# tmoroney/whisper-diarize-rs

Measured on AMD Instinct MI355X. Metric: audio-sec/wall-sec (xRT), large-v3 + DTW + diarize, 1/2/4/8 MI355X, higher is better.
Workload: dtype f16 (f32 accumulate)

## Files before the change

include/wdr.h:

```cpp
#ifndef WDR_H
#define WDR_H

#include <stddef.h>
#include <stdint.h>

#ifdef __cplusplus
extern "C" {
#endif

#define WDR_ABI_VERSION 6

typedef struct wdr_engine wdr_engine;
typedef struct wdr_context wdr_context;

typedef struct {
  const char* cache_dir;
  int8_t enable_dtw;
  int8_t enable_flash_attn;
  int8_t use_gpu;
  int8_t has_gpu_device;
  int32_t gpu_device;
  const char* vad_model_path;
  const char* diarize_segment_model_path;
  const char* diarize_embedding_model_path;
// ... 202 lines not shown
                          uint64_t chunk_frames, int32_t host, int16_t** out, size_t* n_out, double* ms);
int wdr_dbg_audio_split(const uint8_t* raw, uint64_t n_frames, int32_t fmt, int32_t channels, int32_t rate,
                        uint64_t chunk_frames, int32_t host, int16_t** out, size_t* n_per_channel, double* ms);
int wdr_dbg_resample_table(int32_t rate, int32_t* L, int32_t* M, int32_t* T, float** tab);
int wdr_dbg_mfma_scale(const uint8_t* a, const uint8_t* b, const int32_t* sa, const int32_t* sb, float* out);
int wdr_dbg_encode(wdr_context* c, const float* mel_window , float* enc_out );
int wdr_dbg_cross_kv(wdr_context* c, float* out);
int wdr_dbg_decode(wdr_context* c, const int32_t* tokens, size_t n, float* logits_out );
int wdr_dbg_step(wdr_context* c, const int32_t* tokens, size_t n, float* logits_out );
int wdr_dbg_logits(wdr_context* c, const float* logits, int32_t R, const int32_t* ctl, const float* temperature,
                   float max_initial_ts, int32_t suppress_blank, int32_t* ids_out, float* f_out);
int wdr_dbg_batch_step(wdr_context* c, const int32_t* tokens, size_t n, int32_t rows, int32_t iters,
                       double* ms_per_step);
int wdr_dbg_capture(wdr_context* c, const int32_t* tokens, size_t n, float* cap_out );
int wdr_dbg_dtw(const float* cap, int32_t n_heads, int32_t n_tok, int32_t n_audio, int32_t sot_len, int32_t seek,
                float* x_out , int32_t* times_out, int32_t* n_times);
int wdr_dbg_discrete(const float* w, size_t n, uint32_t seed, int32_t n_draws, int32_t* out);
int wdr_dbg_dtw_dp(const float* x, int32_t rows, int32_t cols, int32_t seek, int32_t* times_out, int32_t* n_times);
int wdr_dbg_proj_fp8(const uint16_t* a_f16, const uint16_t* w_f16, const float* bias, int32_t M, int32_t N, int32_t K,
                     int32_t epi, float* out, uint8_t* a8_out, uint8_t* a_scale_out, uint8_t* w8_out,
                     uint8_t* w_scale_out);
int wdr_dbg_proj(const uint16_t* a_f16, const uint16_t* w_f16, const float* bias, int32_t M, int32_t N, int32_t K,
                 int32_t epi, float* out );
#define WDR_DBG_PROJ_ROWS 0x200
#define WDR_DBG_PROJ_GEMM1 0x800
#define WDR_DBG_PROJ_PACKED 0x1000
int wdr_dbg_pack_rows(const uint16_t* w_f16, int32_t N, int32_t K, uint16_t* out);
int wdr_dbg_proj_ln(const float* x, const float* gamma, const float* beta, const uint16_t* w_f16, const float* bias,
                    int32_t M, int32_t N, int32_t K, int32_t epi, int32_t fused, float* out);
int wdr_dbg_attn(const uint16_t* q, const uint16_t* k, const uint16_t* v, int32_t Tq, int32_t Tk, int32_t n_head,
                 int32_t causal, float* out );
int wdr_dbg_xattn(const uint16_t* q, const uint16_t* kv, const int32_t* row_slot, const int32_t* grp, int32_t R,
                  int32_t S, int32_t H, int32_t iters, float* out);

int wdr_dbg_self_attn(const uint16_t* q, const uint16_t* kc, const uint16_t* vc, int32_t n_seq, int32_t T,
                      const int32_t* row_seq, const int32_t* row_pos, int32_t R, int32_t H, float* out);
int wdr_dbg_proj_qkv(const uint16_t* a_f16, const uint16_t* w_f16, const float* bias, int32_t M, int32_t d, int32_t K,
                     const int32_t* row_seq, const int32_t* row_pos, int32_t n_seq, int32_t T, uint16_t* kc_io,
                     uint16_t* vc_io, float* q_out);
int wdr_dbg_proj_qkv_packed(const uint16_t* a_f16, const uint16_t* w_f16, const float* bias, int32_t M, int32_t d,
                            int32_t K, const int32_t* row_seq, const int32_t* row_pos, int32_t n_seq, int32_t T,
                            uint16_t* kc_io, uint16_t* vc_io, float* q_out);
int wdr_dbg_logits_topk(wdr_context* c, const float* logits, int32_t R, const int32_t* ctl, const float* temperature,
                        float max_initial_ts, int32_t suppress_blank, int32_t K, int32_t* ids_out, float* f_out);
int wdr_dbg_logits_probs(wdr_context* c, const float* logits, int32_t R, const int32_t* ctl, const float* temperature,
                         float max_initial_ts, int32_t suppress_blank, float* probs_out, float* logprobs_out);
int wdr_dbg_kv_rows(wdr_context* c, int32_t seq, int32_t n_rows, int32_t write, uint16_t* k, uint16_t* v);
int wdr_dbg_kv_reorder(wdr_context* c, const int32_t* src, const int32_t* dst, int32_t n, int32_t n_rows);

#ifdef __cplusplus
}
#endif
#endif
```

whisper-diarize-rs_amd/csrc/engine.cpp:

```cpp
#include <algorithm>
#include <atomic>
#include <chrono>
#include <cmath>
#include <cstdio>
#include <cstdlib>
#include <cstring>
#include <fstream>
#include <map>
#include <memory>
#include <random>
#include <string>
#include <sys/stat.h>
#include <dirent.h>
#include <condition_variable>
#include <exception>
#include <mutex>
#include <set>
#include <pthread.h>
#include <thread>
#include <vector>

#include "../../include/wdr.h"
#include "audio_file.h"
#include "audio_gpu.h"
// ... 2480 lines not shown
      WDR_HIP(hipMemcpy(h.data(), dout.p, h.size() * 2, hipMemcpyDeviceToHost));
      for (size_t i = 0; i < h.size(); ++i) out[i] = (float)h[i];
    }
    return 0;
  })
}

int wdr_dbg_attn(const uint16_t* q, const uint16_t* k, const uint16_t* v, int32_t Tq, int32_t Tk, int32_t H,
                 int32_t causal, float* out) {
  WDR_GUARD({
    const int d = H * 64;
    DevMem dq((size_t)Tq * d * 2), dk((size_t)Tk * d * 2), dv((size_t)Tk * d * 2), dout((size_t)Tq * d * 2);
    WDR_HIP(hipMemcpy(dq.p, q, dq.bytes, hipMemcpyHostToDevice));
    WDR_HIP(hipMemcpy(dk.p, k, dk.bytes, hipMemcpyHostToDevice));
    WDR_HIP(hipMemcpy(dv.p, v, dv.bytes, hipMemcpyHostToDevice));
    FlashArgs fa{dq.as<f16>(), d, 0, dk.as<f16>(), d, 0, dv.as<f16>(), d, 0, dout.as<f16>(), d, 0, nullptr, Tq, Tk, H,
                 causal, 0.125f};
    DevMem po, pml;
    if (!causal && Tq <= 256 && Tk >= 512) {
      fa.nsplit = 12;
      po = DevMem((size_t)12 * Tq * H * 64 * 4);
      pml = DevMem((size_t)12 * H * Tq * 8);
      fa.part_o = po.as<float>();
      fa.part_ml = pml.as<float2>();
    }
    launch_flash_attn(fa, 1, nullptr);
    std::vector<f16> h((size_t)Tq * d);
    WDR_HIP(hipMemcpy(h.data(), dout.p, h.size() * 2, hipMemcpyDeviceToHost));
    for (size_t i = 0; i < h.size(); ++i) out[i] = (float)h[i];
    return 0;
  })
}

int wdr_dbg_xattn(const uint16_t* q, const uint16_t* kv, const int32_t* row_slot, const int32_t* grp, int32_t R,
                  int32_t S, int32_t H, int32_t iters, float* out) {
  WDR_GUARD({
    WDR_CHECK(R >= 1 && R <= 1024 && S >= 1 && H >= 1 && H <= 32 && iters >= 1, "dbg xattn: bad shape");
    const int d = H * 64, T = 1500;
    DevMem dq((size_t)R * d * 2), dkv((size_t)S * T * 2 * d * 2), dout((size_t)R * d * 2);
    DevMem po((size_t)24 * R * H * 64 * 4), pml((size_t)24 * R * H * 8);
    DevMem drk(R * sizeof(void*)), dg(R * 4), dl(R * 4);
    WDR_HIP(hipMemcpy(dq.p, q, dq.bytes, hipMemcpyHostToDevice));
    WDR_HIP(hipMemcpy(dkv.p, kv, dkv.bytes, hipMemcpyHostToDevice));
    XAttnArgs xa{dq.as<f16>(), d, dkv.as<f16>(), dkv.as<f16>() + d, 2 * d, T, R, H, 0.125f, po.as<float>(),
                 pml.as<float2>(), dout.as<f16>(), d};
    if (row_slot) {
      std::vector<const f16*> rk(R);
      for (int r = 0; r < R; ++r) {
        WDR_CHECK(row_slot[r] >= 0 && row_slot[r] < S, "dbg xattn: slot out of range");
        rk[r] = dkv.as<f16>() + (size_t)row_slot[r] * T * 2 * d;
      }
      WDR_HIP(hipMemcpy(drk.p, rk.data(), R * sizeof(void*), hipMemcpyHostToDevice));
      xa.row_k = drk.as<const f16*>();
      xa.v_off = d;
      bool big = false;
      for (int r = 0; grp && r < R; ++r) big = big || grp[r] > XATTN_GRP_MAX;
      if (grp && big) {
        std::vector<int> g(R, 0), lead;
        std::vector<int4> tiles;
        for (int r = 0; r < R; ++r) {
          if (grp[r] == 0) continue;
          WDR_CHECK(r + grp[r] <= R, "dbg xattn: bad group");
          if (grp[r] <= XATTN_GRP_MAX) {
            g[r] = grp[r];
            lead.push_back(r);
          } else {
            for (int t = 0; t < grp[r]; t += 128) tiles.push_back(make_int4(r + t, std::min(128, grp[r] - t), 1 << 30, 0));
          }
        }
        WDR_HIP(hipMemcpy(dg.p, g.data(), R * 4, hipMemcpyHostToDevice));
        if (!lead.empty()) WDR_HIP(hipMemcpy(dl.p, lead.data(), lead.size() * 4, hipMemcpyHostToDevice));
        DevMem dt(std::max<size_t>(16, tiles.size() * 16));
        if (!tiles.empty()) WDR_HIP(hipMemcpy(dt.p, tiles.data(), tiles.size() * 16, hipMemcpyHostToDevice));
        xa.grp = dg.as<int>();
        xa.lead = dl.as<int>();
        xa.n_vgrp = (int)lead.size();
        xa.vgrp_max = 1;
        for (int r : lead) xa.vgrp_max = std::max(xa.vgrp_max, g[r]);
// ... 1 lines not shown
        xa.n_tiles = (int)tiles.size();
        for (int i = 0; i < iters; ++i) launch_xattn_rows(xa, nullptr);
        WDR_HIP(hipDeviceSynchronize());
        std::vector<f16> h((size_t)R * d);
        WDR_HIP(hipMemcpy(h.data(), dout.p, h.size() * 2, hipMemcpyDeviceToHost));
        for (size_t i = 0; i < h.size(); ++i) out[i] = (float)h[i];
        return 0;
      }
      if (grp) {
        int ng = 0;
        for (int r = 0; r < R; ++r) {
          WDR_CHECK(grp[r] >= 0 && grp[r] <= XATTN_GRP_MAX && r + grp[r] <= R, "dbg xattn: bad group");
          ng += grp[r] > 0;
        }
        WDR_HIP(hipMemcpy(dg.p, grp, R * 4, hipMemcpyHostToDevice));
        xa.grp = dg.as<int>();
        xa.n_grp = ng;
        std::vector<int> lead;
        for (int r = 0; r < R; ++r)
          if (grp[r] > 0) lead.push_back(r);
        WDR_HIP(hipMemcpy(dl.p, lead.data(), lead.size() * 4, hipMemcpyHostToDevice));
        xa.lead = dl.as<int>();
      }
    }
    for (int i = 0; i < iters; ++i) launch_xattn(xa, nullptr);
    WDR_HIP(hipDeviceSynchronize());
    std::vector<f16> h((size_t)R * d);
    WDR_HIP(hipMemcpy(h.data(), dout.p, h.size() * 2, hipMemcpyDeviceToHost));
    for (size_t i = 0; i < h.size(); ++i) out[i] = (float)h[i];
    return 0;
  })
}

static void check_rows(const int32_t* row_seq, const int32_t* row_pos, int R, int n_seq, int T, const char* what) {
  for (int r = 0; r < R; ++r) {
    WDR_CHECK(row_seq[r] >= 0 && row_seq[r] < n_seq, std::string(what) + ": row_seq out of range");
    WDR_CHECK(row_pos[r] >= 0 && row_pos[r] < std::min(T, 448), std::string(what) + ": row_pos out of range");
  }
}

int wdr_dbg_self_attn(const uint16_t* q, const uint16_t* kc, const uint16_t* vc, int32_t n_seq, int32_t T,
                      const int32_t* row_seq, const int32_t* row_pos, int32_t R, int32_t H, float* out) {
  WDR_GUARD({
    WDR_CHECK(q && kc && vc && row_seq && row_pos && out, "dbg self-attn: null argument");
    WDR_CHECK(R >= 1 && R <= 4096 && H >= 1 && H <= 32 && n_seq >= 1 && n_seq <= 64 && T >= 1 && T <= 4096,
              "dbg self-attn: bad shape");
    check_rows(row_seq, row_pos, R, n_seq, T, "dbg self-attn");
    const int d = H * 64;
    const size_t cache = (size_t)n_seq * T * d * 2;
    DevMem dq((size_t)R * d * 2), dk(cache), dv(cache), dout((size_t)R * d * 2), ds(R * 4), dp(R * 4);
    WDR_HIP(hipMemcpy(dq.p, q, dq.bytes, hipMemcpyHostToDevice));
    WDR_HIP(hipMemcpy(dk.p, kc, cache, hipMemcpyHostToDevice));
    WDR_HIP(hipMemcpy(dv.p, vc, cache, hipMemcpyHostToDevice));
    WDR_HIP(hipMemcpy(ds.p, row_seq, R * 4, hipMemcpyHostToDevice));
    WDR_HIP(hipMemcpy(dp.p, row_pos, R * 4, hipMemcpyHostToDevice));
    DecSelfArgs sa{dq.as<f16>(), d, dk.as<f16>(), dv.as<f16>(), (long long)T * d, d, ds.as<int>(), dp.as<int>(),
                   dout.as<f16>(), d, 0.125f};
    launch_dec_self_attn(sa, R, H, nullptr);
    WDR_HIP(hipDeviceSynchronize());
    std::vector<f16> h((size_t)R * d);
    WDR_HIP(hipMemcpy(h.data(), dout.p, h.size() * 2, hipMemcpyDeviceToHost));
    for (size_t i = 0; i < h.size(); ++i) out[i] = (float)h[i];
    return 0;
  })
}

// ... 116 lines not shown
```

whisper-diarize-rs_amd/csrc/kernels/attn.hip:

```cpp
#include <cstdlib>

#include "../common.h"
#include "kernels.h"
#include "../prof.h"

namespace wdr {


constexpr int FA_KB = 64, FA_KS = 72, FA_VS = 68;

template <int OCC>
__global__ __launch_bounds__(256, OCC) void k_flash_attn(FlashArgs a) {
  ProfClock prof_clock_(a.ts);
  __shared__ __attribute__((aligned(16))) f16 Ks[FA_KB * FA_KS];
  __shared__ __attribute__((aligned(16))) f16 Vt[64 * FA_VS];
  const int tid = threadIdx.x, lane = tid & 63, wid = tid >> 6;
  const int qb = blockIdx.x, h = blockIdx.y, b = blockIdx.z;
  const f16* Q = a.q + b * a.q_bs + h * 64;
  const f16* K = a.k + b * a.k_bs + h * a.k_hs;
  const f16* V = a.v + b * a.v_bs + h * a.v_hs;
  if (a.nsplit > 1) Q = a.q + h * 64;
  const int fr = lane & 31, hh = lane >> 5;
  const int qrow = qb * 128 + wid * 32 + fr;
  const int qrow_c = qrow < a.Tq ? qrow : a.Tq - 1;
// ... 115 lines not shown
        o1 = __builtin_amdgcn_mfma_f32_32x32x16_f16(va1, pb, o1, 0, 0, 0);
      }
  }
  if (a.nsplit > 1) {
    if (qrow < a.Tq) {
      float* po = a.part_o + (((long long)b * a.Tq + qrow) * a.n_head + h) * 64;
#pragma unroll
      for (int g = 0; g < 4; ++g) {
        *(float4*)(po + 8 * g + 4 * hh) = make_float4(o0[4 * g], o0[4 * g + 1], o0[4 * g + 2], o0[4 * g + 3]);
        *(float4*)(po + 32 + 8 * g + 4 * hh) = make_float4(o1[4 * g], o1[4 * g + 1], o1[4 * g + 2], o1[4 * g + 3]);
      }
      if (hh == 0) a.part_ml[((long long)b * a.n_head + h) * a.Tq + qrow] = make_float2(m * 0.6931471805599453f, l);
    }
    return;
  }
  if (qrow < a.Tq) {
    const float inv = l > 0.f ? 1.f / l : 0.f;
    f16* O = a.o + b * a.o_bs + (long long)qrow * a.ldo + h * 64;
#pragma unroll
    for (int g = 0; g < 4; ++g) {
      f16x4 w0, w1;
#pragma unroll
      for (int e = 0; e < 4; ++e) {
        w0[e] = (f16)(o0[4 * g + e] * inv);
        w1[e] = (f16)(o1[4 * g + e] * inv);
      }
      *(f16x4*)(O + 8 * g + 4 * hh) = w0;
      *(f16x4*)(O + 32 + 8 * g + 4 * hh) = w1;
    }
    if (a.ml && hh == 0) a.ml[((long long)b * a.n_head + h) * a.Tq + qrow] = make_float2(m * 0.6931471805599453f, l);
  }
}

__global__ __launch_bounds__(64) void k_flash_combine(FlashArgs a) {
  const int q = blockIdx.x, h = blockIdx.y, d = threadIdx.x;
  float2 ml = make_float2(-INFINITY, 0.f);
  if (d < a.nsplit) ml = a.part_ml[((long long)d * a.n_head + h) * a.Tq + q];
  const float M = wave_max(ml.x);
  const float w = (d < a.nsplit && ml.x != -INFINITY) ? __expf(ml.x - M) : 0.f;
  const float L = wave_sum(ml.y * w);
  float acc = 0.f;
  for (int c = 0; c < a.nsplit; ++c) acc += a.part_o[(((long long)c * a.Tq + q) * a.n_head + h) * 64 + d] * __shfl(w, c, 64);
  a.o[(long long)q * a.ldo + h * 64 + d] = (f16)(acc / L);
  if (a.ml && d == 0) a.ml[(long long)h * a.Tq + q] = make_float2(M, L);
}

static int flash_occ() {
  static const int v = getenv("WDR_FLASH_OCC") && atoi(getenv("WDR_FLASH_OCC")) == 4 ? 4 : 3;
  return v;
}

void launch_flash_attn(const FlashArgs& a, int n_batch, hipStream_t s) {
  WDR_CHECK(a.Tq > 0 && a.Tk > 0, "attention: empty");
  auto* kfn = flash_occ() == 4 ? k_flash_attn<4> : k_flash_attn<3>;
  if (a.nsplit > 1) {
    WDR_CHECK(n_batch == 1 && !a.causal && a.nsplit <= 64 && a.part_o && a.part_ml, "flash split: bad args");
    wdr_launch(PROF_FLASH, (double)a.n_head * 64 * 2 * (2.0 * a.Tq + 2.0 * a.Tk), (double)a.n_head * a.Tq * a.Tk * 64 * 4,
               kfn, dim3(cdiv(a.Tq, 128), a.n_head, a.nsplit), dim3(256), 0, s, a);
    WDR_KLAUNCH(k_flash_combine, dim3(a.Tq, a.n_head), dim3(64), 0, s, a);
    WDR_HIP(hipGetLastError());
    return;
  }
  dim3 grid(cdiv(a.Tq, 128), a.n_head, n_batch);
  const double pairs = a.causal ? 0.5 * (double)a.Tq * a.Tk : (double)a.Tq * a.Tk;
  wdr_launch(PROF_FLASH, (double)n_batch * a.n_head * 64 * 2 * (2.0 * a.Tq + 2.0 * a.Tk),
             (double)n_batch * a.n_head * pairs * 64 * 4, kfn, grid, dim3(256), 0, s, a);
  WDR_HIP(hipGetLastError());
}

__global__ __launch_bounds__(256, 8) void k_dec_self_attn(DecSelfArgs a) {
  __shared__ float qs[64];
  __shared__ float sc[448];
  __shared__ float red[2][4];
  __shared__ float po[4][64];
  const int r = blockIdx.x, h = blockIdx.y, tid = threadIdx.x, lane = tid & 63, wid = tid >> 6;
  const int seq = a.row_seq[r];
  const int nk = a.row_pos[r] + 1;
  if (tid < 64) qs[tid] = (float)a.q[(long long)r * a.ldq + h * 64 + tid];
  __syncthreads();
  const f16* K = a.kc + seq * a.seq_stride + h * 64;
  const f16* V = a.vc + seq * a.seq_stride + h * 64;
  float mx = -INFINITY;
  const int kq = tid >> 2, qd = tid & 3;
  float qv[16];
#pragma unroll
  for (int e = 0; e < 16; ++e) qv[e] = qs[qd * 16 + e];
#pragma unroll 1
// ... 201 lines not shown
  for (int hp = 0; hp < 2; ++hp) {
    float acc = 0.f;
#pragma unroll
    for (int i = 0; i < 16; ++i) acc += (float)(f16)ps[hp][wid * 16 + i] * (float)Vs[hp][(wid * 16 + i) * 64 + lane];
    pv[hp][wid][lane] = acc;
  }
  __syncthreads();
  if (tid < 128) {
    const int hp = tid >> 6, dd = tid & 63, h = h0 + hp;
    const long long cr = (long long)c * a.R + r0;
    a.part_o[(cr * a.n_head + h) * 64 + dd] = pv[hp][0][dd] + pv[hp][1][dd] + pv[hp][2][dd] + pv[hp][3][dd];
    if (dd == 0) a.part_ml[cr * a.n_head + h] = make_float2(mx[hp], red[hp][1][0] + red[hp][1][1] + red[hp][1][2] + red[hp][1][3]);
  }
}

template <int NS>
__global__ __launch_bounds__(64) void k_xattn_combine(XAttnArgs a) {
  const int r = blockIdx.x, h = blockIdx.y, d = threadIdx.x;
  float po[NS];
#pragma unroll
  for (int c = 0; c < NS; ++c) po[c] = a.part_o[(((long long)c * a.R + r) * a.n_head + h) * 64 + d];
  float2 ml = make_float2(-INFINITY, 0.f);
  if (d < NS) ml = a.part_ml[((long long)d * a.R + r) * a.n_head + h];
  const float M = wave_max(ml.x);
  const float w = (d < NS && ml.x != -INFINITY) ? __expf(ml.x - M) : 0.f;
  const float L = wave_sum(ml.y * w);
  float acc = 0.f;
#pragma unroll
  for (int c = 0; c < NS; ++c) acc += po[c] * __shfl(w, c, 64);
  a.o[(long long)r * a.ldo + h * 64 + d] = (f16)(acc / L);
  if (a.ml_out && d == 0) a.ml_out[(long long)r * a.n_head + h] = make_float2(M, L);
}

__global__ __launch_bounds__(256) void k_xattn_mma(XAttnArgs a) {
  ProfClock prof_clock_(a.ts);
  __shared__ __attribute__((aligned(16))) f16 Ks[FA_KB * FA_KS];
  __shared__ __attribute__((aligned(16))) f16 Vt[64 * FA_VS];
  const int c = blockIdx.x, h = blockIdx.y, tid = threadIdx.x, lane = tid & 63, wid = tid >> 6;
  const int4 t = a.tiles[blockIdx.z];
  if (a.layer >= t.z) return;
  const f16* kb = a.row_k[t.x] + a.layer_off + h * a.hs;
  const f16* vb = kb + a.v_off;
  const int key0 = c * FA_KB;
#pragma unroll
  for (int i = 0; i < 2; ++i) {
    const int e = tid + 256 * i;
    const int r = e >> 3, col = (e & 7) * 8;
    int key = key0 + r;
    key = key < a.Tk ? key : a.Tk - 1;
    const f16x8 kr = *(const f16x8*)(kb + (long long)key * a.ldkv + col);
    const f16x8 vr = *(const f16x8*)(vb + (long long)key * a.ldkv + col);
    *(f16x8*)(Ks + r * FA_KS + col) = kr;
#pragma unroll
    for (int j = 0; j < 8; ++j) Vt[(col + j) * FA_VS + r] = vr[j];
  }
  __syncthreads();
  if (32 * wid >= t.y) return;
  const int fr = lane & 31, hh = lane >> 5;
  const int ql = 32 * wid + fr;
  const int qrow = t.x + (ql < t.y ? ql : t.y - 1);
  f16x8 qf[4];
#pragma unroll
  for (int s4 = 0; s4 < 4; ++s4) qf[s4] = *(const f16x8*)(a.q + (long long)qrow * a.ldq + h * 64 + 16 * s4 + 8 * hh);
  f32x16 st[2];
#pragma unroll
  for (int u = 0; u < 2; ++u) {
#pragma unroll
    for (int r = 0; r < 16; ++r) st[u][r] = 0.f;
#pragma unroll
    for (int s4 = 0; s4 < 4; ++s4) {
      const f16x8 af = *(const f16x8*)(Ks + (32 * u + fr) * FA_KS + 16 * s4 + 8 * hh);
      st[u] = __builtin_amdgcn_mfma_f32_32x32x16_f16(af, qf[s4], st[u], 0, 0, 0);
    }
  }
  float mx = -INFINITY;
#pragma unroll
  for (int u = 0; u < 2; ++u)
#pragma unroll
    for (int r = 0; r < 16; ++r) {
      const int key = key0 + 32 * u + (r & 3) + 8 * (r >> 2) + 4 * hh;
      const float sv = key < a.Tk ? st[u][r] * a.scale : -INFINITY;
      st[u][r] = sv;
      mx = fmaxf(mx, sv);
    }
  mx = fmaxf(mx, __shfl_xor(mx, 32, 64));
  float rs = 0.f;
#pragma unroll
  for (int u = 0; u < 2; ++u)
#pragma unroll
    for (int r = 0; r < 16; ++r) {
      const float p = st[u][r] == -INFINITY ? 0.f : __expf(st[u][r] - mx);
      st[u][r] = p;
      rs += p;
    }
  rs += __shfl_xor(rs, 32, 64);
  f32x16 o0, o1;
#pragma unroll
  for (int r = 0; r < 16; ++r) { o0[r] = 0.f; o1[r] = 0.f; }
#pragma unroll
  for (int u = 0; u < 2; ++u)
#pragma unroll
    for (int s2 = 0; s2 < 2; ++s2) {
      f16x8 pb;
#pragma unroll
      for (int j = 0; j < 8; ++j) pb[j] = (f16)st[u][8 * s2 + j];
      const int kc = 32 * u + 16 * s2 + 4 * hh;
      const f16x4 lo0 = *(const f16x4*)(Vt + fr * FA_VS + kc), hi0 = *(const f16x4*)(Vt + fr * FA_VS + kc + 8);
      const f16x4 lo1 = *(const f16x4*)(Vt + (32 + fr) * FA_VS + kc), hi1 = *(const f16x4*)(Vt + (32 + fr) * FA_VS + kc + 8);
      const f16x8 va0 = {lo0[0], lo0[1], lo0[2], lo0[3], hi0[0], hi0[1], hi0[2], hi0[3]};
      const f16x8 va1 = {lo1[0], lo1[1], lo1[2], lo1[3], hi1[0], hi1[1], hi1[2], hi1[3]};
      o0 = __builtin_amdgcn_mfma_f32_32x32x16_f16(va0, pb, o0, 0, 0, 0);
      o1 = __builtin_amdgcn_mfma_f32_32x32x16_f16(va1, pb, o1, 0, 0, 0);
    }
  if (ql >= t.y) return;
  const long long cr = (long long)c * a.R + t.x + ql;
  float* po = a.part_o + (cr * a.n_head + h) * 64;
#pragma unroll
  for (int g = 0; g < 4; ++g) {
    *(float4*)(po + 8 * g + 4 * hh) = make_float4(o0[4 * g], o0[4 * g + 1], o0[4 * g + 2], o0[4 * g + 3]);
    *(float4*)(po + 32 + 8 * g + 4 * hh) = make_float4(o1[4 * g], o1[4 * g + 1], o1[4 * g + 2], o1[4 * g + 3]);
  }
  if (hh == 0) a.part_ml[cr * a.n_head + h] = make_float2(mx, rs);
}

void launch_xattn_rows(const XAttnArgs& a, hipStream_t s) {
  WDR_CHECK(cdiv(a.Tk, XA_KC) == XA_NS && XA_KC == FA_KB, "cross-attention rows expect 1500 keys");
  WDR_CHECK(a.row_k && a.R >= 1 && (a.n_vgrp == 0 || (a.grp && a.lead)) && (a.n_tiles == 0 || a.tiles),
            "cross-attention rows: bad tables");
  const double kv = (double)a.Tk * a.n_head * 64 * 2 * 2;
  if (a.n_vgrp > 0) {
    const double flops = (double)a.R * a.Tk * a.n_head * 64 * 4;
    if (a.vgrp_max <= 1 && a.n_head % 2 == 0)
      wdr_launch(PROF_XATTN, a.n_vgrp * kv, flops, k_xattn_partial2, dim3(XA_NS, a.n_head / 2, a.n_vgrp), dim3(256),
                 0, s, a);
    else if (a.vgrp_max <= 1)
      wdr_launch(PROF_XATTN, a.n_vgrp * kv, flops, k_xattn_partial<true, 1>, dim3(XA_NS, a.n_head, a.n_vgrp),
                 dim3(256), 0, s, a);
    else
      wdr_launch(PROF_XATTN, a.n_vgrp * kv, flops, k_xattn_partial<true, XATTN_GRP_MAX>,
                 dim3(XA_NS, a.n_head, a.n_vgrp), dim3(256), 0, s, a);
  }
  if (a.n_tiles > 0)
    wdr_launch(PROF_XATTN, a.n_tiles * kv, (double)a.n_tiles * 128 * a.Tk * a.n_head * 64 * 4, k_xattn_mma,
               dim3(XA_NS, a.n_head, a.n_tiles), dim3(256), 0, s, a);
  WDR_KLAUNCH(k_xattn_combine<XA_NS>, dim3(a.R, a.n_head), dim3(64), 0, s, a);
  WDR_HIP(hipGetLastError());
}

void launch_xattn(const XAttnArgs& a, hipStream_t s) {
  WDR_CHECK(cdiv(a.Tk, XA_KC) == XA_NS, "cross-attention decode expects 1500 keys");
  WDR_CHECK(a.R >= 1 && (a.row_k || a.R <= XATTN_GRP_MAX), "cross-attention decode: R out of range");
  const int ng = a.row_k ? (a.grp ? a.n_grp : a.R) : 1;
  const double bytes = (double)ng * a.Tk * a.n_head * 64 * 2 * 2, flops = (double)a.R * a.Tk * a.n_head * 64 * 4;
  WDR_CHECK(!a.lead || (a.grp && a.n_grp >= 1 && a.n_grp <= a.R), "cross-attention decode: leaders need groups");
  if (a.row_k && !a.grp && a.n_head % 2 == 0)
    wdr_launch(PROF_XATTN, bytes, flops, k_xattn_partial2, dim3(XA_NS, a.n_head / 2, a.R), dim3(256), 0, s, a);
  else if (a.row_k && !a.grp)
    wdr_launch(PROF_XATTN, bytes, flops, k_xattn_partial<true, 1>, dim3(XA_NS, a.n_head, a.R), dim3(256), 0, s, a);
  else if (a.row_k)
    wdr_launch(PROF_XATTN, bytes, flops, k_xattn_partial<true, XATTN_GRP_MAX>,
               dim3(XA_NS, a.n_head, a.lead ? a.n_grp : a.R), dim3(256), 0, s, a);
  else
    wdr_launch(PROF_XATTN, bytes, flops, k_xattn_partial<false, XATTN_GRP_MAX>, dim3(XA_NS, a.n_head), dim3(256), 0,
               s, a);
  WDR_KLAUNCH(k_xattn_combine<XA_NS>, dim3(a.R, a.n_head), dim3(64), 0, s, a);
  WDR_HIP(hipGetLastError());
}


__global__ __launch_bounds__(256) void k_aheads_capture_rows(CaptureRowsArgs a) {
  __shared__ float qs[64];
  const int j = blockIdx.x, i = blockIdx.y, tid = threadIdx.x;
  const int r = a.crow[j], h = a.heads[i];
  if (tid < 64) qs[tid] = (float)a.q[(long long)r * a.ldq + h * 64 + tid];
  __syncthreads();
  const float2 ml = a.ml[(long long)r * a.n_head + h];
  const float inv = 1.f / ml.y;
// ... 23 lines not shown
```

whisper-diarize-rs_amd/csrc/kernels/kernels.h:

```cpp
#pragma once
#include "../common.h"

namespace wdr {

struct MelArgs {
  const float* x; int n;
  int n_frames;
  int n_mels;
  const float* hann;
  const float* cos_tab; const float* sin_tab;
  const float* filters;
  float* mel;
  int* gmax;
};
void launch_mel(const MelArgs& a, hipStream_t s);
void launch_gmax_init(int* gmax, hipStream_t s);

struct Im2colMelArgs {
  const float* mel; int n_mels, n_fft_frames;
  const int* gmax;
  int seek;
  int kp;
  f16* out;
};
// ... 39 lines not shown
struct TokOut {
  int id, tid;
  float p, plog, pt, ptsum;
  float nosp_prob;
  int pad;
};
void launch_logits_topk(const float* logits, int ld, const LogitsCtl* ctls, const VocabIds& v, int R, int K,
                        float* work, BeamCand* out, hipStream_t s);
void launch_logits_probs(const float* logits, int ld, const LogitsCtl* ctls, const VocabIds& v, int R, float* work,
                         float* probs, float* logprobs, hipStream_t s);
void launch_kv_copy(f16* kc, f16* vc, long long seq_stride, int nslot, int L, const int* pairs_dev, int n_pairs,
                    int n_rows, int d, hipStream_t s);
void launch_logits_process(const float* logits, int ld, const LogitsCtl* ctls, const VocabIds& v, int R, float* work,
                           TokOut* out, hipStream_t s);

void launch_dtw(const float* cap, int A, int N_tok, int Tk, int n_audio, int sot_len, int seek, float* nrm, float* x,
                int* times, int* n_times, hipStream_t s);
void launch_dtw_dp_only(const float* x, int rows, int M, int seek, int* times, int* n_times, hipStream_t s);

struct FlashArgs {
  const f16* q; int ldq; long long q_bs;
  const f16* k; int ldk; long long k_bs;
  const f16* v; int ldv; long long v_bs;
  f16* o; int ldo; long long o_bs;
  float2* ml;
  int Tq, Tk, n_head;
  int causal;
  float scale;
  long long k_hs = 64, v_hs = 64;
  int nsplit = 1;
  float* part_o = nullptr;
  float2* part_ml = nullptr;
  unsigned long long* ts = nullptr;
};
inline unsigned long long* prof_attach(FlashArgs& a) { return a.ts = prof_slot(); }
void launch_flash_attn(const FlashArgs& a, int n_batch, hipStream_t s);
struct DecSelfArgs {
  const f16* q; int ldq;
  const f16* kc; const f16* vc;
  long long seq_stride; int d;
  const int* row_seq; const int* row_pos;
  f16* o; int ldo;
  float scale;
};
void launch_dec_self_attn(const DecSelfArgs& a, int R, int n_head, hipStream_t s);
struct XAttnArgs {
  const f16* q; int ldq;
  const f16* k; const f16* v; int ldkv;
  int Tk, R, n_head;
  float scale;
  float* part_o;
  float2* part_ml;
  f16* o; int ldo;
  const f16* const* row_k = nullptr;
  long long layer_off = 0;
  long long v_off = 0;
  long long hs = 64;
  unsigned long long* ts = nullptr;
  const int* grp = nullptr;
  int n_grp = 0;
  const int* lead = nullptr;
  int layer = 0;
  const int* lend = nullptr;
  const int4* tiles = nullptr;
  int n_tiles = 0;
  int n_vgrp = 0;
  int vgrp_max = 1;
  float2* ml_out = nullptr;
};
constexpr int XATTN_GRP_MAX = 8;
inline unsigned long long* prof_attach(XAttnArgs& a) { return a.ts = prof_slot(); }
void launch_xattn(const XAttnArgs& a, hipStream_t s);
void launch_xattn_rows(const XAttnArgs& a, hipStream_t s);
struct CaptureRowsArgs {
  const f16* q; int ldq;
  const f16* const* row_k; long long layer_off, hs;
  const float2* ml;
  const int* heads;
  const int* crow; float* const* cdst; const int* cstride;
  int n_cap, slot0, Tk, n_head;
  float scale;
};
void launch_aheads_capture_rows(const CaptureRowsArgs& a, int n_sel, hipStream_t s);
void launch_layernorm_rows(const float* x, int ldx, const float* g, const float* b, f16* y, int ldy, int rows, int d,
                           const int* row_map, hipStream_t s);

struct VadWeights {
  const f16* stft;
  const f16* c0w; const float* c0b;
  const f16* c1w; const float* c1b;
  const f16* c2w; const float* c2b;
  const f16* c3w; const float* c3b;
  const f16* wih; const float* bih;
  const f16* whh; const float* bhh;
  const f16* wo;  const float* bo;
};
void launch_vad(const float* x, long long n, const VadWeights& w, float* xg, float* hout, float* probs,
                hipStream_t s);

enum Act : int { ACT_NONE = 0, ACT_RELU = 1, ACT_LRELU = 2, ACT_SIGMOID = 3, ACT_ABS = 4 };
struct Gemm32Args {
// ... 46 lines not shown
```

whisper-diarize-rs_amd/wdr/_lib.py:

```python
from __future__ import annotations

import atexit
import ctypes as C
import os
import re

PKG_DIR = os.path.dirname(os.path.dirname(os.path.abspath(__file__)))
LIB_PATH = os.environ.get("WDR_AB_LIB") or os.path.join(PKG_DIR, "libwdr.so")
HEADER = os.path.join(os.path.dirname(PKG_DIR), "include", "wdr.h")

i8, i32, i64, u64 = C.c_int8, C.c_int32, C.c_int64, C.c_uint64
f32, f64, cstr, vp, sz = C.c_float, C.c_double, C.c_char_p, C.c_void_p, C.c_size_t


class EngineConfig(C.Structure):
    _fields_ = [("cache_dir", cstr), ("enable_dtw", i8), ("enable_flash_attn", i8), ("use_gpu", i8),
                ("has_gpu_device", i8), ("gpu_device", i32), ("vad_model_path", cstr),
                ("diarize_segment_model_path", cstr), ("diarize_embedding_model_path", cstr)]


class Advanced(C.Structure):
    _fields_ = [("sampling_strategy", cstr), ("has_best_of_or_beam_size", i8), ("best_of_or_beam_size", i32),
                ("has_n_threads", i8), ("n_threads", i32), ("has_temperature", i8), ("temperature", f32),
                ("has_max_text_ctx", i8), ("max_text_ctx", i32), ("init_prompt", cstr),
# ... 133 lines not shown
    "wdr_ggml_info": (C.c_int, [cstr, P(i32), P(i64), P(i64)]),
    "wdr_ggml_tensor_types": (C.c_int, [cstr, P(i64)]),
    "wdr_ggml_tensor_f16": (C.c_int, [cstr, cstr, P(P(C.c_uint16)), P(sz)]),
    "wdr_dbg_dequant": (C.c_int, [i32, P(C.c_uint8), sz, P(C.c_uint16), P(f64)]),
    "wdr_dbg_batch_step": (C.c_int, [vp, P(i32), sz, i32, i32, P(f64)]),
    "wdr_context_stage_times": (C.c_int, [vp, P(StageTimes)]),
    "wdr_context_hparams": (C.c_int, [vp, P(i32)]),
    "wdr_prof_set": (C.c_int, [i32]),
    "wdr_prof_read": (C.c_int, [P(f64), P(i64), P(f64), P(f64)]),
    "wdr_prof_set_mask": (C.c_int, [i32]),
    "wdr_prof_read_class": (C.c_int, [i32, P(f64), P(i64), P(f64), P(f64)]),
    "wdr_prof_read_clock": (C.c_int, [i32, P(f64), P(i64), P(f64), P(f64)]),
    "wdr_state_full": (C.c_int, [vp, P(f32), sz, P(TranscribeOptions), P(Synthetic), cstr, P(P(ResultSeg)), P(sz),
                                 P(i32)]),
    "wdr_result_free": (None, [P(ResultSeg), sz]),
    "wdr_dbg_log_mel": (C.c_int, [vp, P(f32), sz, i32, P(f32)]),
    "wdr_dbg_energy": (C.c_int, [P(f32), sz, P(f32)]),
    "wdr_dbg_mfma_scale": (C.c_int, [P(C.c_uint8), P(C.c_uint8), P(i32), P(i32), P(f32)]),
    "wdr_dbg_encode": (C.c_int, [vp, P(f32), P(f32)]),
    "wdr_dbg_decode": (C.c_int, [vp, P(i32), sz, P(f32)]),
    "wdr_dbg_cross_kv": (C.c_int, [vp, P(f32)]),
    "wdr_dbg_step": (C.c_int, [vp, P(i32), sz, P(f32)]),
    "wdr_dbg_logits": (C.c_int, [vp, P(f32), i32, P(i32), P(f32), f32, i32, P(i32), P(f32)]),
    "wdr_dbg_capture": (C.c_int, [vp, P(i32), sz, P(f32)]),
    "wdr_dbg_dtw": (C.c_int, [P(f32), i32, i32, i32, i32, i32, P(f32), P(i32), P(i32)]),
    "wdr_dbg_discrete": (C.c_int, [P(f32), sz, C.c_uint32, i32, P(i32)]),
    "wdr_dbg_dtw_dp": (C.c_int, [P(f32), i32, i32, i32, P(i32), P(i32)]),
    "wdr_dbg_proj": (C.c_int, [P(C.c_uint16), P(C.c_uint16), P(f32), i32, i32, i32, i32, P(f32)]),
    "wdr_dbg_proj_ln": (C.c_int, [P(f32), P(f32), P(f32), P(C.c_uint16), P(f32), i32, i32, i32, i32, i32, P(f32)]),
    "wdr_dbg_proj_fp8": (C.c_int, [P(C.c_uint16), P(C.c_uint16), P(f32), i32, i32, i32, i32, P(f32), P(C.c_uint8),
                                   P(C.c_uint8), P(C.c_uint8), P(C.c_uint8)]),
    "wdr_dbg_attn": (C.c_int, [P(C.c_uint16), P(C.c_uint16), P(C.c_uint16), i32, i32, i32, i32, P(f32)]),
    "wdr_dbg_xattn": (C.c_int, [P(C.c_uint16), P(C.c_uint16), P(i32), P(i32), i32, i32, i32, i32, P(f32)]),
    "wdr_dbg_self_attn": (C.c_int, [P(C.c_uint16), P(C.c_uint16), P(C.c_uint16), i32, i32, P(i32), P(i32), i32, i32,
                                    P(f32)]),
    "wdr_dbg_proj_qkv": (C.c_int, [P(C.c_uint16), P(C.c_uint16), P(f32), i32, i32, i32, P(i32), P(i32), i32, i32,
                                   P(C.c_uint16), P(C.c_uint16), P(f32)]),
    "wdr_dbg_proj_qkv_packed": (C.c_int, [P(C.c_uint16), P(C.c_uint16), P(f32), i32, i32, i32, P(i32), P(i32), i32,
                                          i32, P(C.c_uint16), P(C.c_uint16), P(f32)]),
    "wdr_dbg_pack_rows": (C.c_int, [P(C.c_uint16), i32, i32, P(C.c_uint16)]),
    "wdr_dbg_logits_topk": (C.c_int, [vp, P(f32), i32, P(i32), P(f32), f32, i32, i32, P(i32), P(f32)]),
    "wdr_dbg_logits_probs": (C.c_int, [vp, P(f32), i32, P(i32), P(f32), f32, i32, P(f32), P(f32)]),
    "wdr_dbg_kv_rows": (C.c_int, [vp, i32, i32, i32, P(C.c_uint16), P(C.c_uint16)]),
    "wdr_dbg_kv_reorder": (C.c_int, [vp, P(i32), P(i32), i32, i32]),
}

_lib = None


class WdrError(RuntimeError):
    pass


def header_symbols():
    txt = open(HEADER).read()
    return sorted(set(re.findall(r"\b(wdr_[a-z0-9_]+)\s*\(", txt)))


def load():
    global _lib
    if _lib is not None:
        return _lib
    if not os.path.exists(LIB_PATH):
        raise WdrError("libwdr.so not built at %s (run __graft_entry__.build())" % LIB_PATH)
    lib = C.CDLL(LIB_PATH)
    for name, (res, args) in _SIGS.items():
# ... 12 lines not shown
```

Baseline: 905.4.

## Use LDS transpose reads for V fragments in flash and cross attention

Adds a new non-causal flash-attention kernel that stores V row-major in LDS with an XOR swizzle. It builds the PV MFMA operands with ds_read_tr16_b64 transpose loads, where the old kernel did a scalar transposing scatter into LDS. The same path is offered as a template variant of the cross-attention MMA kernel, gated by the WDR_ATTN_TR level. It is on by default for encoder flash attention (level 1) and opt-in for cross-attention (level 2). The change also restructures double-buffered K/V prefetch, relying on gfx950-only transpose LDS reads and new swizzle indexing that could be wrong.

```diff
diff --git a/include/wdr.h b/include/wdr.h
--- a/include/wdr.h
+++ b/include/wdr.h
@@ -258,6 +258,10 @@
                  int32_t causal, float* out );
 int wdr_dbg_xattn(const uint16_t* q, const uint16_t* kv, const int32_t* row_slot, const int32_t* grp, int32_t R,
                   int32_t S, int32_t H, int32_t iters, float* out);
+int wdr_dbg_attn_qkv(const uint16_t* qkv, int32_t n_batch, int32_t Tq, int32_t Tk, int32_t n_head, int32_t variant,
+                     uint16_t* out);
+int wdr_dbg_xattn_variant(const uint16_t* q, const uint16_t* kv, const int32_t* row_slot, const int32_t* grp,
+                          int32_t R, int32_t S, int32_t H, int32_t variant, float* out);
 
 int wdr_dbg_self_attn(const uint16_t* q, const uint16_t* kc, const uint16_t* vc, int32_t n_seq, int32_t T,
                       const int32_t* row_seq, const int32_t* row_pos, int32_t R, int32_t H, float* out);
diff --git a/whisper-diarize-rs_amd/csrc/engine.cpp b/whisper-diarize-rs_amd/csrc/engine.cpp
--- a/whisper-diarize-rs_amd/csrc/engine.cpp
+++ b/whisper-diarize-rs_amd/csrc/engine.cpp
@@ -2536,8 +2536,29 @@
   })
 }
 
-int wdr_dbg_xattn(const uint16_t* q, const uint16_t* kv, const int32_t* row_slot, const int32_t* grp, int32_t R,
-                  int32_t S, int32_t H, int32_t iters, float* out) {
+int wdr_dbg_attn_qkv(const uint16_t* qkv, int32_t n_batch, int32_t Tq, int32_t Tk, int32_t H, int32_t variant,
+                     uint16_t* out) {
+  WDR_GUARD({
+    WDR_CHECK(n_batch >= 1 && n_batch <= 64 && Tq >= 1 && Tk >= 1 && Tq <= 4096 && Tk <= 4096 && H >= 1 && H <= 32,
+              "dbg attn qkv: bad shape");
+    WDR_CHECK(variant == 0 || variant == 1, "dbg attn qkv: variant is 0 or 1");
+    const int d = H * 64, T = std::max(Tq, Tk);
+    const long long bs = (long long)T * 3 * d, obs = (long long)Tq * d;
+    DevMem dqkv((size_t)n_batch * bs * 2), dout((size_t)n_batch * obs * 2);
+    WDR_HIP(hipMemcpy(dqkv.p, qkv, dqkv.bytes, hipMemcpyHostToDevice));
+    f16* A = dqkv.as<f16>();
+    FlashArgs fa{A, 3 * d, bs, A + d, 3 * d, bs, A + 2 * d, 3 * d, bs, dout.as<f16>(), d, obs, nullptr, Tq, Tk, H,
+                 0, 0.125f};
+    fa.tr = variant;
+    launch_flash_attn(fa, n_batch, nullptr);
+    WDR_HIP(hipDeviceSynchronize());
+    WDR_HIP(hipMemcpy(out, dout.p, dout.bytes, hipMemcpyDeviceToHost));
+    return 0;
+  })
+}
+
+static int dbg_xattn_run(const uint16_t* q, const uint16_t* kv, const int32_t* row_slot, const int32_t* grp, int32_t R,
+                         int32_t S, int32_t H, int32_t iters, int tr, float* out) {
   WDR_GUARD({
     WDR_CHECK(R >= 1 && R <= 1024 && S >= 1 && H >= 1 && H <= 32 && iters >= 1, "dbg xattn: bad shape");
     const int d = H * 64, T = 1500;
@@ -2548,6 +2569,7 @@
     WDR_HIP(hipMemcpy(dkv.p, kv, dkv.bytes, hipMemcpyHostToDevice));
     XAttnArgs xa{dq.as<f16>(), d, dkv.as<f16>(), dkv.as<f16>() + d, 2 * d, T, R, H, 0.125f, po.as<float>(),
                  pml.as<float2>(), dout.as<f16>(), d};
+    xa.tr = tr;
     if (row_slot) {
       std::vector<const f16*> rk(R);
       for (int r = 0; r < R; ++r) {
@@ -2615,6 +2637,17 @@
   })
 }
 
+int wdr_dbg_xattn(const uint16_t* q, const uint16_t* kv, const int32_t* row_slot, const int32_t* grp, int32_t R,
+                  int32_t S, int32_t H, int32_t iters, float* out) {
+  return dbg_xattn_run(q, kv, row_slot, grp, R, S, H, iters, -1, out);
+}
+
+int wdr_dbg_xattn_variant(const uint16_t* q, const uint16_t* kv, const int32_t* row_slot, const int32_t* grp,
+                          int32_t R, int32_t S, int32_t H, int32_t variant, float* out) {
+  WDR_GUARD({ WDR_CHECK(variant == 0 || variant == 1, "dbg xattn: variant is 0 or 1"); })
+  return dbg_xattn_run(q, kv, row_slot, grp, R, S, H, 1, variant, out);
+}
+
 static void check_rows(const int32_t* row_seq, const int32_t* row_pos, int R, int n_seq, int T, const char* what) {
   for (int r = 0; r < R; ++r) {
     WDR_CHECK(row_seq[r] >= 0 && row_seq[r] < n_seq, std::string(what) + ": row_seq out of range");
diff --git a/whisper-diarize-rs_amd/csrc/kernels/attn.hip b/whisper-diarize-rs_amd/csrc/kernels/attn.hip
--- a/whisper-diarize-rs_amd/csrc/kernels/attn.hip
+++ b/whisper-diarize-rs_amd/csrc/kernels/attn.hip
@@ -171,6 +171,182 @@
   }
 }
 
+constexpr int FA_VR = 64;
+__device__ __forceinline__ int v_tr_col(int key, int col) { return col ^ (((key >> 1) & 1) << 5); }
+__device__ __forceinline__ f16x4 lds_read_tr(const f16* p) {
+  typedef __fp16 h16x4 __attribute__((__vector_size__(4 * sizeof(__fp16))));
+  return __builtin_bit_cast(f16x4, __builtin_amdgcn_ds_read_tr16_b64_v4f16((__attribute__((address_space(3))) h16x4*)p));
+}
+__device__ __forceinline__ int v_tr_base(int lane) {
+  const int q = (lane & 15) >> 2, key = 4 * (lane >> 5) + q;
+  return key * FA_VR + v_tr_col(key, 16 * ((lane >> 4) & 1) + 4 * (lane & 3));
+}
+__device__ __forceinline__ void v_tr_frag(const f16* Vs, int vb, int kc0, f16x8& va0, f16x8& va1) {
+  const f16x4 lo0 = lds_read_tr(Vs + kc0 * FA_VR + vb), hi0 = lds_read_tr(Vs + (kc0 + 8) * FA_VR + vb);
+  const f16x4 lo1 = lds_read_tr(Vs + kc0 * FA_VR + (vb ^ 32)), hi1 = lds_read_tr(Vs + (kc0 + 8) * FA_VR + (vb ^ 32));
+  va0 = (f16x8){lo0[0], lo0[1], lo0[2], lo0[3], hi0[0], hi0[1], hi0[2], hi0[3]};
+  va1 = (f16x8){lo1[0], lo1[1], lo1[2], lo1[3], hi1[0], hi1[1], hi1[2], hi1[3]};
+}
+
+__global__ __launch_bounds__(256, 3) void k_flash_attn_tr(FlashArgs a) {
+  ProfClock prof_clock_(a.ts);
+  __shared__ __attribute__((aligned(16))) f16 Ks[2][FA_KB * FA_KS];
+  __shared__ __attribute__((aligned(16))) f16 Vs[2][FA_KB * FA_VR];
+  const int tid = threadIdx.x, lane = tid & 63, wid = tid >> 6;
+  const int qb = blockIdx.x, h = blockIdx.y, b = blockIdx.z;
+  const f16* Q = a.q + b * a.q_bs + h * 64;
+  const f16* K = a.k + b * a.k_bs + h * a.k_hs;
+  const f16* V = a.v + b * a.v_bs + h * a.v_hs;
+  const int fr = lane & 31, hh = lane >> 5;
+  const int qrow = qb * 128 + wid * 32 + fr;
+  const int qrow_c = qrow < a.Tq ? qrow : a.Tq - 1;
+
+  f16x8 qf[4];
+#pragma unroll
+  for (int s = 0; s < 4; ++s) qf[s] = *(const f16x8*)(Q + (long long)qrow_c * a.ldq + 16 * s + 8 * hh);
+
+  f32x16 o0, o1;
+#pragma unroll
+  for (int r = 0; r < 16; ++r) { o0[r] = 0.f; o1[r] = 0.f; }
+  float m = -INFINITY, l = 0.f;
+  const int kmax = a.Tk;
+  f16x8 kreg[2], vreg[2];
+  const int sr = 2 * (tid >> 3), scol = (tid & 7) * 8;
+  auto load_rows = [&](const f16* P, int ld, int kt, f16x8 (&reg)[2]) {
+#pragma unroll
+    for (int i = 0; i < 2; ++i) {
+      int key = kt + sr + i;
+      key = key < kmax ? key : kmax - 1;
+      reg[i] = *(const f16x8*)(P + (long long)key * ld + scol);
+    }
+  };
+  const int ksto = sr * FA_KS + scol, vsto = sr * FA_VR + v_tr_col(sr, scol);
+  auto store_k = [&](int buf) {
+#pragma unroll
+    for (int i = 0; i < 2; ++i) *(f16x8*)(Ks[buf] + ksto + i * FA_KS) = kreg[i];
+  };
+  auto store_v = [&](int buf) {
+#pragma unroll
+    for (int i = 0; i < 2; ++i) *(f16x8*)(Vs[buf] + vsto + i * FA_VR) = vreg[i];
+  };
+  const int kb = fr * FA_KS + 8 * hh, vb = v_tr_base(lane);
+  auto qk = [&](int buf, f32x16 (&st)[2]) {
+#pragma unroll
+    for (int t = 0; t < 2; ++t) {
+#pragma unroll
+      for (int r = 0; r < 16; ++r) st[t][r] = 0.f;
+#pragma unroll
+      for (int s = 0; s < 4; ++s) {
+        const f16x8 af = *(const f16x8*)(Ks[buf] + kb + 32 * t * FA_KS + 16 * s);
+        st[t] = __builtin_amdgcn_mfma_f32_32x32x16_f16(af, qf[s], st[t], 0, 0, 0);
+      }
+    }
+  };
+  const float sl2 = a.scale * 1.4426950408889634f;
+  auto tile = [&](int k0, int buf, f32x16 (&st)[2], f32x16 (&sn)[2]) {
+    __syncthreads();
+    if (k0 + FA_KB < kmax) store_v(buf ^ 1);
+    if (k0 + 2 * FA_KB < kmax) {
+      store_k(buf);
+      load_rows(V, a.ldv, k0 + 2 * FA_KB, vreg);
+      if (k0 + 3 * FA_KB < kmax) load_rows(K, a.ldk, k0 + 3 * FA_KB, kreg);
+    }
+    float mx = -INFINITY;
+    if (k0 + FA_KB <= kmax) {
+#pragma unroll
+      for (int t = 0; t < 2; ++t)
+#pragma unroll
+        for (int r = 0; r < 16; ++r) mx = fmaxf(mx, st[t][r]);
+    } else {
+#pragma unroll
+      for (int t = 0; t < 2; ++t)
+#pragma unroll
+        for (int r = 0; r < 16; ++r) {
+          const int key = k0 + 32 * t + (r & 3) + 8 * (r >> 2) + 4 * hh;
+          st[t][r] = key < kmax ? st[t][r] : -INFINITY;
+          mx = fmaxf(mx, st[t][r]);
+        }
+    }
+    mx = fmaxf(mx, __shfl_xor(mx, 32, 64));
+    const float mnew = fmaxf(m, mx == -INFINITY ? -INFINITY : mx * sl2);
+    const float alpha = (mnew == -INFINITY) ? 1.f : __builtin_amdgcn_exp2f(m - mnew);
+    const float mu = (mnew == -INFINITY) ? 0.f : mnew;
+    qk(buf ^ 1, sn);
+    float rs = 0.f;
+#pragma unroll
+    for (int t = 0; t < 2; ++t)
+#pragma unroll
+      for (int r = 0; r < 16; ++r) {
+        const float p = __builtin_amdgcn_exp2f(__builtin_fmaf(st[t][r], sl2, -mu));
+        st[t][r] = p;
+        rs += p;
+      }
+#pragma unroll
+    for (int i = 0; i < 8; ++i) {
+      __builtin_amdgcn_sched_group_barrier(0x008, 1, 0);
+      __builtin_amdgcn_sched_group_barrier(0x002, 12, 0);
+    }
+    rs += __shfl_xor(rs, 32, 64);
+    l = l * alpha + rs;
+    const bool moved = __any(mnew != m);
+    m = mnew;
+    if (moved) {
+#pragma unroll
+      for (int r = 0; r < 16; ++r) { o0[r] *= alpha; o1[r] *= alpha; }
+    }
+#pragma unroll
+    for (int t = 0; t < 2; ++t)
+#pragma unroll
+      for (int s = 0; s < 2; ++s) {
+        f16x8 pb;
+#pragma unroll
+        for (int j = 0; j < 8; ++j) pb[j] = (f16)st[t][8 * s + j];
+        f16x8 va0, va1;
+        v_tr_frag(Vs[buf], vb, 32 * t + 16 * s, va0, va1);
+        o0 = __builtin_amdgcn_mfma_f32_32x32x16_f16(va0, pb, o0, 0, 0, 0);
+        o1 = __builtin_amdgcn_mfma_f32_32x32x16_f16(va1, pb, o1, 0, 0, 0);
+      }
+  };
+  load_rows(K, a.ldk, 0, kreg);
+  load_rows(V, a.ldv, 0, vreg);
+  __builtin_amdgcn_s_waitcnt(0x0f70);
+  store_k(0);
+  store_v(0);
+  if (FA_KB < kmax) {
+    load_rows(K, a.ldk, FA_KB, kreg);
+    load_rows(V, a.ldv, FA_KB, vreg);
+  }
+  __syncthreads();
+  f32x16 sa[2], sb[2];
+  qk(0, sa);
+  if (FA_KB < kmax) {
+    store_k(1);
+    if (2 * FA_KB < kmax) load_rows(K, a.ldk, 2 * FA_KB, kreg);
+  }
+  for (int k0 = 0;;) {
+    tile(k0, 0, sa, sb);
+    if ((k0 += FA_KB) >= kmax) break;
+    tile(k0, 1, sb, sa);
+    if ((k0 += FA_KB) >= kmax) break;
+  }
+  if (qrow < a.Tq) {
+    const float inv = l > 0.f ? 1.f / l : 0.f;
+    f16* O = a.o + b * a.o_bs + (long long)qrow * a.ldo + h * 64;
+#pragma unroll
+    for (int g = 0; g < 4; ++g) {
+      f16x4 w0, w1;
+#pragma unroll
+      for (int e = 0; e < 4; ++e) {
+        w0[e] = (f16)(o0[4 * g + e] * inv);
+        w1[e] = (f16)(o1[4 * g + e] * inv);
+      }
+      *(f16x4*)(O + 8 * g + 4 * hh) = w0;
+      *(f16x4*)(O + 32 + 8 * g + 4 * hh) = w1;
+    }
+    if (a.ml && hh == 0) a.ml[((long long)b * a.n_head + h) * a.Tq + qrow] = make_float2(m * 0.6931471805599453f, l);
+  }
+}
+
 __global__ __launch_bounds__(64) void k_flash_combine(FlashArgs a) {
   const int q = blockIdx.x, h = blockIdx.y, d = threadIdx.x;
   float2 ml = make_float2(-INFINITY, 0.f);
@@ -189,9 +365,16 @@
   return v;
 }
 
+static int attn_tr_level() {
+  static const int v = getenv("WDR_ATTN_TR") ? atoi(getenv("WDR_ATTN_TR")) : 1;
+  return v;
+}
+
 void launch_flash_attn(const FlashArgs& a, int n_batch, hipStream_t s) {
   WDR_CHECK(a.Tq > 0 && a.Tk > 0, "attention: empty");
   auto* kfn = flash_occ() == 4 ? k_flash_attn<4> : k_flash_attn<3>;
+  if (!a.causal && a.nsplit <= 1 && flash_occ() != 4 && (a.tr < 0 ? attn_tr_level() >= 1 : a.tr != 0))
+    kfn = k_flash_attn_tr;
   if (a.nsplit > 1) {
     WDR_CHECK(n_batch == 1 && !a.causal && a.nsplit <= 64 && a.part_o && a.part_ml, "flash split: bad args");
     wdr_launch(PROF_FLASH, (double)a.n_head * 64 * 2 * (2.0 * a.Tq + 2.0 * a.Tk), (double)a.n_head * a.Tq * a.Tk * 64 * 4,
@@ -459,10 +642,11 @@
   if (a.ml_out && d == 0) a.ml_out[(long long)r * a.n_head + h] = make_float2(M, L);
 }
 
+template <bool TR>
 __global__ __launch_bounds__(256) void k_xattn_mma(XAttnArgs a) {
   ProfClock prof_clock_(a.ts);
   __shared__ __attribute__((aligned(16))) f16 Ks[FA_KB * FA_KS];
-  __shared__ __attribute__((aligned(16))) f16 Vt[64 * FA_VS];
+  __shared__ __attribute__((aligned(16))) f16 Vt[TR ? FA_KB * FA_VR : 64 * FA_VS];
   const int c = blockIdx.x, h = blockIdx.y, tid = threadIdx.x, lane = tid & 63, wid = tid >> 6;
   const int4 t = a.tiles[blockIdx.z];
   if (a.layer >= t.z) return;
@@ -478,8 +662,12 @@
     const f16x8 kr = *(const f16x8*)(kb + (long long)key * a.ldkv + col);
     const f16x8 vr = *(const f16x8*)(vb + (long long)key * a.ldkv + col);
     *(f16x8*)(Ks + r * FA_KS + col) = kr;
-#pragma unroll
-    for (int j = 0; j < 8; ++j) Vt[(col + j) * FA_VS + r] = vr[j];
+    if (TR) {
+      *(f16x8*)(Vt + r * FA_VR + v_tr_col(r, col)) = vr;
+    } else {
+#pragma unroll
+      for (int j = 0; j < 8; ++j) Vt[(col + j) * FA_VS + r] = vr[j];
+    }
   }
   __syncthreads();
   if (32 * wid >= t.y) return;
@@ -531,11 +719,16 @@
       f16x8 pb;
 #pragma unroll
       for (int j = 0; j < 8; ++j) pb[j] = (f16)st[u][8 * s2 + j];
-      const int kc = 32 * u + 16 * s2 + 4 * hh;
-      const f16x4 lo0 = *(const f16x4*)(Vt + fr * FA_VS + kc), hi0 = *(const f16x4*)(Vt + fr * FA_VS + kc + 8);
-      const f16x4 lo1 = *(const f16x4*)(Vt + (32 + fr) * FA_VS + kc), hi1 = *(const f16x4*)(Vt + (32 + fr) * FA_VS + kc + 8);
-      const f16x8 va0 = {lo0[0], lo0[1], lo0[2], lo0[3], hi0[0], hi0[1], hi0[2], hi0[3]};
-      const f16x8 va1 = {lo1[0], lo1[1], lo1[2], lo1[3], hi1[0], hi1[1], hi1[2], hi1[3]};
+      f16x8 va0, va1;
+      if (TR) {
+        v_tr_frag(Vt, v_tr_base(lane), 32 * u + 16 * s2, va0, va1);
+      } else {
+        const int kc = 32 * u + 16 * s2 + 4 * hh;
+        const f16x4 lo0 = *(const f16x4*)(Vt + fr * FA_VS + kc), hi0 = *(const f16x4*)(Vt + fr * FA_VS + kc + 8);
+        const f16x4 lo1 = *(const f16x4*)(Vt + (32 + fr) * FA_VS + kc), hi1 = *(const f16x4*)(Vt + (32 + fr) * FA_VS + kc + 8);
+        va0 = (f16x8){lo0[0], lo0[1], lo0[2], lo0[3], hi0[0], hi0[1], hi0[2], hi0[3]};
+        va1 = (f16x8){lo1[0], lo1[1], lo1[2], lo1[3], hi1[0], hi1[1], hi1[2], hi1[3]};
+      }
       o0 = __builtin_amdgcn_mfma_f32_32x32x16_f16(va0, pb, o0, 0, 0, 0);
       o1 = __builtin_amdgcn_mfma_f32_32x32x16_f16(va1, pb, o1, 0, 0, 0);
     }
@@ -568,8 +761,9 @@
                  dim3(XA_NS, a.n_head, a.n_vgrp), dim3(256), 0, s, a);
   }
   if (a.n_tiles > 0)
-    wdr_launch(PROF_XATTN, a.n_tiles * kv, (double)a.n_tiles * 128 * a.Tk * a.n_head * 64 * 4, k_xattn_mma,
-               dim3(XA_NS, a.n_head, a.n_tiles), dim3(256), 0, s, a);
+    wdr_launch(PROF_XATTN, a.n_tiles * kv, (double)a.n_tiles * 128 * a.Tk * a.n_head * 64 * 4,
+               (a.tr < 0 ? attn_tr_level() >= 2 : a.tr != 0) ? k_xattn_mma<true> : k_xattn_mma<false>, dim3(XA_NS, a.n_head, a.n_tiles), dim3(256), 0,
+               s, a);
   WDR_KLAUNCH(k_xattn_combine<XA_NS>, dim3(a.R, a.n_head), dim3(64), 0, s, a);
   WDR_HIP(hipGetLastError());
 }
diff --git a/whisper-diarize-rs_amd/csrc/kernels/kernels.h b/whisper-diarize-rs_amd/csrc/kernels/kernels.h
--- a/whisper-diarize-rs_amd/csrc/kernels/kernels.h
+++ b/whisper-diarize-rs_amd/csrc/kernels/kernels.h
@@ -95,6 +95,7 @@
   float* part_o = nullptr;
   float2* part_ml = nullptr;
   unsigned long long* ts = nullptr;
+  int tr = -1;
 };
 inline unsigned long long* prof_attach(FlashArgs& a) { return a.ts = prof_slot(); }
 void launch_flash_attn(const FlashArgs& a, int n_batch, hipStream_t s);
@@ -130,6 +131,7 @@
   int n_vgrp = 0;
   int vgrp_max = 1;
   float2* ml_out = nullptr;
+  int tr = -1;
 };
 constexpr int XATTN_GRP_MAX = 8;
 inline unsigned long long* prof_attach(XAttnArgs& a) { return a.ts = prof_slot(); }
diff --git a/whisper-diarize-rs_amd/wdr/_lib.py b/whisper-diarize-rs_amd/wdr/_lib.py
--- a/whisper-diarize-rs_amd/wdr/_lib.py
+++ b/whisper-diarize-rs_amd/wdr/_lib.py
@@ -189,6 +189,8 @@
                                    P(C.c_uint8), P(C.c_uint8), P(C.c_uint8)]),
     "wdr_dbg_attn": (C.c_int, [P(C.c_uint16), P(C.c_uint16), P(C.c_uint16), i32, i32, i32, i32, P(f32)]),
     "wdr_dbg_xattn": (C.c_int, [P(C.c_uint16), P(C.c_uint16), P(i32), P(i32), i32, i32, i32, i32, P(f32)]),
+    "wdr_dbg_attn_qkv": (C.c_int, [P(C.c_uint16), i32, i32, i32, i32, i32, P(C.c_uint16)]),
+    "wdr_dbg_xattn_variant": (C.c_int, [P(C.c_uint16), P(C.c_uint16), P(i32), P(i32), i32, i32, i32, i32, P(f32)]),
     "wdr_dbg_self_attn": (C.c_int, [P(C.c_uint16), P(C.c_uint16), P(C.c_uint16), i32, i32, P(i32), P(i32), i32, i32,
                                     P(f32)]),
     "wdr_dbg_proj_qkv": (C.c_int, [P(C.c_uint16), P(C.c_uint16), P(f32), i32, i32, i32, P(i32), P(i32), i32, i32,
```

Result: no change. 910.6, median of 5 (+0.6%).
